# sriramelango/optimized-diffusion-model

Measured on AMD Instinct MI355X. Metric: trajectories/sec (1000-step PC sampler, NCSN++ [1,9,9], bs=128/GPU), higher is better.
Workload: dtype f32; 1 GPU; NCSN++ nf=64 ch_mult=[1,2,2] on [128,1,9,9] per GPU, 1000-step reflected PC sampler (predictor euler_maruyama, corrector none), classifier-free guidance on (2B-sample forwards), fp32; global_batch=128, num_scales=1000, score_evals_per_traj=999, parallelism=single GPU

## Files before the change

### optimized-diffusion-model_amd/csrc/misc_kernels.h

```cpp
#pragma once
#include "common.h"

struct PackJob {
    const float* src;
    float* dst;
    int Cin, Cout;
    int Kpad;
    int Npad;
    int n_off;
    int ntap;
    long s_co, s_ci, s_t;
    int kind;
    const float* src2;
    int col_il;
};

__global__ __launch_bounds__(RDMI_THREADS) void pack_kernel(const PackJob* __restrict__ jobs) {
    const PackJob j = jobs[blockIdx.y];
    const int stride = gridDim.x * RDMI_THREADS;
    if (j.kind == 1) {
        for (int i = blockIdx.x * RDMI_THREADS + threadIdx.x; i < j.Cout; i += stride) j.dst[j.n_off + i] = j.src[i];
        return;
    }
    if (j.kind == 4) {
// ... 201 lines not shown
};

__global__ __launch_bounds__(RDMI_THREADS) void em_update_kernel(
    const float* __restrict__ x, const float* __restrict__ score, const float* __restrict__ zbase,
    const float* __restrict__ t_vec, const float* __restrict__ ts, const StepState* __restrict__ st,
    float* __restrict__ x_out, float* __restrict__ x_mean_out, float* __restrict__ trace,
    int B, int E, int N, float smin, float ratio, float gconst, int z_by_draw) {
    const long i = (long)blockIdx.x * RDMI_THREADS + threadIdx.x;
    if (i >= (long)B * E) return;
    const float t = t_vec ? t_vec[i / E] : ts[st->step];
    const float sigma = smin * powf(ratio, t);
    const float g = sigma * gconst;
    const float dt = -1.0f / (float)N;
    const float* z = z_by_draw ? zbase + (long)st->draw * B * E : zbase;
    const float drift = 0.0f - (g * g) * score[i];
    const float xm = x[i] + drift * dt;
    const float xn = xm + (g * sqrtf(-dt)) * z[i];
    const float xr = reflect_f(xn);
    x_out[i] = xr;
    if (x_mean_out) x_mean_out[i] = reflect_f(xm);
    if (trace) trace[(long)st->step * B * E + i] = xr;
}

__global__ __launch_bounds__(RDMI_THREADS) void em_fused_kernel(
    const float* __restrict__ x, const float* __restrict__ s, const float* __restrict__ w, const float* __restrict__ z,
    float* __restrict__ x_out, float* __restrict__ trace, const float* __restrict__ teacher,
    int B, int E, int N, float t, float smin, float ratio, float gconst, int use_cfg, uint64_t seed, uint64_t elem_offset, uint32_t draw) {
    const long i = (long)blockIdx.x * RDMI_THREADS + threadIdx.x;
    if (i >= (long)B * E) return;
    float score = s[i];
    if (use_cfg) { const float wt = w ? w[i / E] : 0.f; score = (1.0f + wt) * score - wt * s[(long)B * E + i]; }
    float zz;
    if (z) zz = z[i];
    else { const uint64_t g = elem_offset + (uint64_t)i; zz = philox_normal4(seed, g >> 2, draw)[(int)(g & 3)]; }
    const float sigma = smin * powf(ratio, t);
    const float g_ = sigma * gconst;
    const float dt = -1.0f / (float)N;
    const float drift = 0.0f - (g_ * g_) * score;
    const float xm = x[i] + drift * dt;
    const float xr = reflect_f(xm + (g_ * sqrtf(-dt)) * zz);
    if (trace) trace[i] = xr;
    x_out[i] = teacher ? teacher[i] : xr;
}

__global__ __launch_bounds__(64) void langevin_prep_kernel(
    const float* __restrict__ s, const float* __restrict__ w, const float* __restrict__ z_in, float* __restrict__ score_out,
    float* __restrict__ z_out, float* __restrict__ norms, int B, int E, int use_cfg, uint64_t seed, uint64_t elem_offset, uint32_t draw) {
    const int b = blockIdx.x, lane = threadIdx.x;
    const float wt = (use_cfg && w) ? w[b] : 0.f;
    float s2 = 0.f, z2 = 0.f;
    for (int e = lane; e < E; e += 64) {
        const long i = (long)b * E + e;
        float sc = s[i];
        if (use_cfg) sc = (1.0f + wt) * sc - wt * s[(long)B * E + i];
        float zz;
        if (z_in) zz = z_in[i];
        else { const uint64_t g = elem_offset + (uint64_t)i; zz = philox_normal4(seed, g >> 2, draw)[(int)(g & 3)]; }
        score_out[i] = sc; z_out[i] = zz;
        s2 += sc * sc; z2 += zz * zz;
    }
    for (int m = 32; m >= 1; m >>= 1) { s2 += __shfl_xor(s2, m); z2 += __shfl_xor(z2, m); }
    if (lane == 0) { norms[b] = sqrtf(s2); norms[B + b] = sqrtf(z2); }
}
// ... 211 lines not shown
```

### optimized-diffusion-model_amd/csrc/rdmi.hip

```cpp
#include <hip/hip_runtime.h>

#include <algorithm>
#include <cmath>
#include <cstdarg>
#include <cstdio>
#include <cstdlib>
#include <cstring>
#include <climits>
#include <map>
#include <memory>
#include <stdexcept>
#include <string>
#include <vector>

#include "../../include/rdmi.h"
#include "attn_kernel.h"
#include "conv_kernel.h"
#include "misc_kernels.h"
#include "unet_kernel.h"
#include "bwd_kernels.h"
#include "opt_kernels.h"
#include "ode_kernels.h"
#include "tiled_kernels.h"

// ... 119 lines not shown
    dev_ptr<float> d_w;
    size_t w_floats = 0;
    dev_ptr<int> d_int;
    dev_ptr<float> ws;
    size_t ws_per_sample = 0;
    size_t w_t0 = 0, w_t2 = 0, w_dense = 0, b_dense = 0;
    dev_ptr<float> d_h1, d_temb, d_dense;
    dev_ptr<float> d_s2, d_score, d_z, d_norms, d_ts, d_tvec;
    dev_ptr<float> d_tt, d_th1; int tt_cap = 0;
    dev_ptr<float> d_dense_all; size_t dense_all_cap = 0;
    dev_ptr<StepState> d_state;
    bool use_fused = true;
    dev_ptr<long long> d_stamps;
    struct FPatch { int op; int field; std::string param; size_t arena_off; };
    struct FusedProg {
        int S = 1; bool ok = false; std::string why;
        std::vector<FOp> fprog;
        std::vector<FPatch> fpatch; std::vector<short> ftabs;
        std::vector<std::string> fdesc;
        dev_ptr<FOp> d_fprog; dev_ptr<short> d_ftabs; dev_ptr<float> d_spill; size_t spill_per_sample = 0;
        UnetArgs fargs{}; size_t fused_lds = 0;
        bool coop = false; int n_xchg = 0; dev_ptr<unsigned long long> d_xbuf; dev_ptr<int> d_coop_err; int max_nb = 0;
        bool train = false;
    };
    std::unique_ptr<TiledPlan> tiled;
    bool in_train_forward = false;
    dev_ptr<bf16_t> d_w16;
    std::vector<FusedProg> progs;
    int s_min_wg = 256;
    bool use_coop = true;
    int coop_stride = 1;
    unsigned coop_epoch = 0;
    int last_prog = 0;
    const FusedProg* pick(int NB) const {
        if (use_coop) for (auto& q : progs) if (q.ok && q.coop && !q.train && NB <= q.max_nb) return &q;
        const FusedProg* best = nullptr;
        for (auto& q : progs) if (q.ok && !q.coop && !q.train && (q.S == 1 || NB >= s_min_wg * q.S) && (!best || q.S > best->S)) best = &q;
        return best;
    }
    bool fused_ready() const { return !progs.empty() && progs[0].ok; }
    float train_drop_p = 0.f; const unsigned long long* train_seed_dev = nullptr;
    int train_prog = -1;
    std::map<std::string, size_t> wmap;
    bool packed_valid = false;
    bool debug_taps = false;
    bool profiling = false;
    std::vector<ProfEntry> prof;
    std::vector<std::pair<hipEvent_t, hipEvent_t>> ev_pool;
    std::vector<int> ev_entry;
    size_t ev_used = 0;
    std::unique_ptr<TrainPlan> train;
    ~rdmi_ctx();
};

namespace {
// ... 978 lines not shown

int resident_workgroups() {
#ifdef RDMI_EMU
    return 256;
#else
    int dev = 0, cus = 0;
    if (hipGetDevice(&dev) != hipSuccess || hipDeviceGetAttribute(&cus, hipDeviceAttributeMultiprocessorCount, dev) != hipSuccess) return 0;
    return cus;
#endif
}

int build_fused_program(rdmi_ctx* c) {
    if (int e = build_one_program(c, 1)) return e;
    const char* only = std::getenv("RDMI_S");
    if (const char* e = std::getenv("RDMI_S_MIN_WG")) c->s_min_wg = std::max(1, atoi(e));
    for (int S : {2, 4})
        if (c->progs[0].ok && c->arch.n_levels >= 2 && c->max_batch >= c->s_min_wg * S && (!only || atoi(only) >= S))
            if (int e = build_one_program(c, S)) return e;
    if (const char* e = std::getenv("RDMI_COOP")) c->use_coop = atoi(e) != 0;
#ifdef RDMI_EMU
    c->coop_stride = 1;
#endif
    if (const char* e = std::getenv("RDMI_COOP_STRIDE")) c->coop_stride = std::max(1, atoi(e));
    if (c->progs[0].ok && c->use_coop && c->arch.n_levels >= 2 && !only)
        if (int e = build_one_program(c, 4, true)) return e;
    return 0;
}

int build_fused_program_pass(rdmi_ctx* c, rdmi_ctx::FusedProg& q, int S, int TAB_RESERVE, int TAB1_RESERVE, int* tab_used, int* tab1_used, bool coop, bool train) {
    using LT = FusedBuilder::LT;
    const rdmi_arch& a = c->arch;
    q.S = S; q.train = train;
    FusedBuilder b{c, q};
    b.S = S; b.coop = coop; b.train = train;
    if (train) {
        for (size_t i = 0; i < c->tensors.size(); ++i) b.lp_tensor[c->tensors[i].name] = (int)i;
        for (size_t i = 0; i < c->ops.size(); ++i) b.lp_op[c->ops[i].name] = (int)i;
    }
    const int nslot0 = coop ? 1 : S;
    Layout L = build_layout(c);
    std::map<std::string, int> dense_off;
    {
        int dt = 0;
        for (auto& d : L.down) { dense_off[d.name] = dt; dt += d.cout; }
        dense_off["mid_block1"] = dt; dt += L.mid_ch;
        dense_off["mid_block2"] = dt; dt += L.mid_ch;
// ... 213 lines not shown
        FOp& o = q.fprog[(size_t)f.op];
        float* p = q.d_spill.get() + f.off * (size_t)spill_n;
        if (f.which == 1) o.b_g = p; else if (f.which == 2) o.a_g = p; else o.g_out = p;
    }
    UnetArgs& fa = q.fargs;
    fa = UnetArgs{};
    fa.prog = q.d_fprog.get(); fa.nops = (int)q.fprog.size();
    fa.tabs = q.d_ftabs.get(); fa.tab_bytes = (int)(tab0_shorts * sizeof(short)); fa.tab_base = 0;
    if (loadtab_idx >= 0) q.fprog[(size_t)loadtab_idx].a_g = reinterpret_cast<const float*>(q.d_ftabs.get() + tab0_shorts);
    fa.zero_off = TAB_RESERVE; fa.zero_bytes = zero_bytes;
    fa.dense = c->d_dense.get(); fa.dense_stride = c->dense_total; fa.S = S;
    fa.out_elems = c->H * c->W * a.channels;
    if (coop) {
        const int groups_max = ceil_div(coop_max_nb, 4);
        const size_t xb = (size_t)groups_max * 2 * 4 * (size_t)b.xslot_granules * sizeof(unsigned long long);
        HIP_OK(hip_alloc(q.d_xbuf, std::max<size_t>(xb, 16) / sizeof(unsigned long long)));
        HIP_OK(hipMemset(q.d_xbuf.get(), 0, std::max<size_t>(xb, 16)));
        HIP_OK(hip_alloc(q.d_coop_err, 4));
        HIP_OK(hipMemset(q.d_coop_err.get(), 0, 16));
        fa.coop = 1; fa.coop_stride = c->coop_stride; fa.xbuf = q.d_xbuf.get(); fa.xslot = b.xslot_granules;
        fa.coop_err = q.d_coop_err.get();
        if (const char* e = std::getenv("RDMI_COOP_TEST_BREAK")) fa.coop_break = atoi(e);
        q.coop = true; q.n_xchg = b.n_xchg; q.max_nb = coop_max_nb;
    }
    q.fused_lds = (size_t)b.high_water;
    if (const char* e = std::getenv("RDMI_UDBG")) fa.dbg = atoi(e);
    if (std::getenv("RDMI_STAMPS") && (S == 1 || coop)) {
        if (!c->d_stamps) HIP_OK(hip_alloc(c->d_stamps, 1024 + 200 * 8 + 8));
        if (q.fprog.size() > 200) return fail("RDMI_STAMPS: program of %zu ops", q.fprog.size());
        fa.stamps = c->d_stamps.get();
    }
    q.fdesc.clear();
    for (auto& o : q.fprog) {
        char buf[160];
        const char* kn[] = {"GATHER", "STORE", "GN", "CONV", "ATTN", "LOADTAB", "XCHG"};
        if (o.kind == FOP_CONV) snprintf(buf, sizeof buf, "CONV rows=%d mtiles=%d K=%dx%d(+%d) Cout=%d dst=%d%s", o.rows, o.mtiles, o.ntap, o.main_ph.nch * 16, o.nsc ? o.sc[0].nch * 16 : 0, o.Cout, o.dst_kind, o.gn_off >= 0 ? (o.gn_raw ? (o.coop ? " +GN(copy) coop" : " +GN(copy)") : (o.coop ? " +GN coop" : " +GN")) : (o.coop ? " coop" : ""));
        else snprintf(buf, sizeof buf, "%s rows=%d C=%d", kn[o.kind], o.rows, o.C);
        q.fdesc.push_back(buf);
    }
    q.ok = true;
    return 0;
}

struct ProfScope {
    rdmi_ctx* c; hipStream_t s; int entry = -1; size_t slot = 0;
    ProfScope(rdmi_ctx* c_, hipStream_t s_, const std::string& name, double flops) : c(c_), s(s_) {
// ... 116 lines not shown
                case FusedBuilder::F_BIAS2: o.bias2 = p; break;
                case FusedBuilder::F_W: o.main_ph.w = p; break;
                case FusedBuilder::F_SC0W: o.sc[0].w = p; break;
                case FusedBuilder::F_SC1W: o.sc[1].w = p; break;
            }
        }
        HIP_OK(hipMemcpyAsync(q.d_fprog.get(), q.fprog.data(), q.fprog.size() * sizeof(FOp), hipMemcpyHostToDevice, s));
    }
    if (c->fused_ready()) HIP_OK(hipStreamSynchronize(s));
    c->packed_valid = true;
    return 0;
}

struct FwdIn {
    const float* x; int x_mod;
    const float* sig; int sig_mod;
    float t_scalar;
    int t_is_time; float smin, ratio;
    const float* labels; int label_rows;
    float* out; int NB;
    const float* tt_row = nullptr;
    const float* dense_rows = nullptr;
    float drop_p = 0.f; const unsigned long long* seed_dev = nullptr;
};

}
#include "tiled_plan.h"
namespace {

int run_forward(rdmi_ctx* c, const FwdIn& f, hipStream_t s) {
    const rdmi_arch& a = c->arch;
    if (f.NB < 1 || f.NB > c->max_batch) return fail("batch %d outside [1, %d] (rdmi_create max_batch)", f.NB, c->max_batch);
    if (a.scale_by_sigma && !c->tiled) return fail("scale_by_sigma=True is only built for the tiled plan (the shipped GTO-Halo config sets it False, RD/configs/model/ncsnpp.yaml)");
    if (a.conditional && !f.labels) return fail("class_labels is required: the model is conditional (label_emb) -- reference raises here too (RD/models/ncsnpp.py:262)");
    const int T = c->temb, Np_t = (T + 63) & ~63, Np_d = (c->dense_total + 63) & ~63;
    if (!f.tt_row && !f.dense_rows) {
    LinArgs l{};
    l.M = f.NB; l.fourW = P(c, "time_embed.W"); l.nfour = a.nf;
    l.X = f.sig; l.x_mod = f.sig_mod > 0 ? f.sig_mod : f.NB; l.t_is_time = f.t_is_time; l.smin = f.smin; l.ratio = f.ratio;
    l.use_scalar = f.sig ? 0 : 1; l.t_scalar = f.t_scalar;
    l.pre = 2; l.K = pad16(2 * a.nf); l.W = c->d_w.get() + c->w_t0; l.Npad = Np_t; l.N = T; l.bias = P(c, "time_mlp.0.bias");
    l.Y = c->d_h1.get(); l.ldy = T;
    {
        ProfScope ps(c, s, "linear_mfma(time_mlp.0)", 2.0 * f.NB * T * 2 * a.nf);
        hipLaunchKernelGGL(linear_mfma_kernel<1>, dim3((unsigned)ceil_div(f.NB, 16), (unsigned)(Np_t / 64)), dim3(RDMI_THREADS), 0, s, l);
    }
// ... 18 lines not shown
        ProfScope ps(c, s, "linear_mfma(Dense_0 x all)", 2.0 * f.NB * T * c->dense_total);
        hipLaunchKernelGGL((linear_mfma_kernel<1, 16>), dim3((unsigned)ceil_div(f.NB, 16), (unsigned)(Np_d / 64)), dim3(RDMI_THREADS), 0, s, l3);
    }
    }
    HIP_OK(hipGetLastError());
    if (a.compute_dtype == 1 && !c->tiled && !c->in_train_forward)
        return fail("compute_dtype=bf16 on this shape is built for the TRAINING step only (model.train_dtype = 'bf16'); sampling and evaluation of the "
                    "GTO-Halo model run the exact-fp32 plans");
    if (c->tiled) return run_tiled(c, f, s);
    const rdmi_ctx::FusedProg* fq = (c->use_fused && !c->debug_taps) ? c->pick(f.NB) : nullptr;
    if (c->in_train_forward) {
        static const int fused_upto = [] { const char* e = std::getenv("RDMI_TRAIN_FUSED_UPTO"); return e ? atoi(e) : 2 * std::max(resident_workgroups(), 1); }();
        fq = (c->train_prog >= 0 && c->progs[(size_t)c->train_prog].ok && f.NB <= fused_upto) ? &c->progs[(size_t)c->train_prog] : nullptr;
    }
    if (fq) {
        static bool attr_set = false;
        if (!attr_set) {
            HIP_OK(hipFuncSetAttribute(reinterpret_cast<const void*>(unet_wg_kernel<false>), hipFuncAttributeMaxDynamicSharedMemorySize, 160 * 1024));
            HIP_OK(hipFuncSetAttribute(reinterpret_cast<const void*>(unet_wg_kernel<true>), hipFuncAttributeMaxDynamicSharedMemorySize, 160 * 1024));
            HIP_OK(hipFuncSetAttribute(reinterpret_cast<const void*>((unet_wg_kernel<false, true>)), hipFuncAttributeMaxDynamicSharedMemorySize, 160 * 1024));
            HIP_OK(hipFuncSetAttribute(reinterpret_cast<const void*>((unet_wg_kernel<false, true, true>)), hipFuncAttributeMaxDynamicSharedMemorySize, 160 * 1024));
            HIP_OK(hipFuncSetAttribute(reinterpret_cast<const void*>((unet_wg_kernel<true, true, true>)), hipFuncAttributeMaxDynamicSharedMemorySize, 160 * 1024));
            HIP_OK(hipFuncSetAttribute(reinterpret_cast<const void*>((unet_wg_kernel<false, false, false, true>)), hipFuncAttributeMaxDynamicSharedMemorySize, 160 * 1024));
            attr_set = true;
        }
        UnetArgs ua = fq->fargs;
        ua.x_in = f.x; ua.x_mod = f.x_mod; ua.out = f.out; ua.NB = f.NB;
        unsigned nwg = (unsigned)ceil_div(f.NB, fq->S);
        if (fq->coop) {
            nwg = (unsigned)(ceil_div(ceil_div(f.NB, 4), ua.coop_stride) * 4 * ua.coop_stride);
            ua.epoch_base = c->coop_epoch;
            c->coop_epoch += (unsigned)fq->n_xchg;
            if (c->coop_epoch > 0xfff00000u) c->coop_epoch = 0;
        }
        if (f.dense_rows) ua.dense = f.dense_rows;
        double fl = 0;
        for (auto& op : c->ops) fl += op.flops_per_sample;
        ProfScope ps(c, s, "unet_wg_kernel", fl * f.NB);
        c->last_prog = (int)(fq - c->progs.data());
        if (fq->train) {
            ua.drop_p = c->train_drop_p; ua.seed_dev = c->train_seed_dev;
            hipLaunchKernelGGL((unet_wg_kernel<false, false, false, true>), dim3(nwg), dim3(UW_THREADS), fq->fused_lds, s, ua);
            HIP_OK(hipGetLastError());
            return 0;
        }
        if ((ua.stamps || ua.dbg) && fq->S == 1) hipLaunchKernelGGL(unet_wg_kernel<true>, dim3(nwg), dim3(UW_THREADS), fq->fused_lds, s, ua);
        else if ((ua.stamps || ua.dbg) && fq->coop) hipLaunchKernelGGL((unet_wg_kernel<true, true, true>), dim3(nwg), dim3(UW_THREADS), fq->fused_lds, s, ua);
        else if (fq->coop) hipLaunchKernelGGL((unet_wg_kernel<false, true, true>), dim3(nwg), dim3(UW_THREADS), fq->fused_lds, s, ua);
        else if (fq->S > 1) hipLaunchKernelGGL((unet_wg_kernel<false, true>), dim3(nwg), dim3(UW_THREADS), fq->fused_lds, s, ua);
        else hipLaunchKernelGGL(unet_wg_kernel<false>, dim3(nwg), dim3(UW_THREADS), fq->fused_lds, s, ua);
        HIP_OK(hipGetLastError());
        return 0;
    }
    for (auto& op : c->ops) {
        if (op.kind == OP_CONV) {
            ConvArgs ca = op.conv;
            ca.NB = f.NB;
            if (op.a_is_input) { ca.srcA = f.x; ca.srcA_mod = f.x_mod; }
            if (op.out_is_output) ca.out = f.out;
            if (op.use_dense && f.dense_rows) ca.dense = f.dense_rows;
            ProfScope ps(c, s, cfg_name(op.cfg), op.flops_per_sample * f.NB);
            if (int e = launch_conv(op.cfg, ca, s)) return e;
        } else {
            AttnArgs aa = op.attn;
            aa.NB = f.NB;
            ProfScope ps(c, s, "attn_mfma<64>", op.flops_per_sample * f.NB);
            if (int e = launch_attn(aa, s)) return e;
        }
    }
// ... 60 lines not shown
    if (it == c->wmap.end()) return fail("no packed tensor '%s'", key);
    if (it->second + numel > c->w_floats) return fail("packed tensor '%s': %zu floats exceed the arena", key, numel);
    HIP_OK(hipMemcpyAsync(dst, c->d_w.get() + it->second, numel * sizeof(float), hipMemcpyDeviceToDevice, (hipStream_t)stream));
    return 0;
}

const char* rdmi_path_info(rdmi_ctx* c) {
    static thread_local std::string s;
    if (!c) return "";
    if (c->tiled) {
        s = std::string("tiled (") + (c->arch.compute_dtype == 1 ? "bf16 MFMA operands, fp32 accumulate" : "fp32") + "): " + std::to_string(c->tiled->launches.size()) + " launches over HBM-resident NHWC tensors (" + std::to_string(c->tiled->ws_per_sample * 4 / 1024) + " KiB of activations per sample)";
        long n_resize = 0;
        for (auto& l : c->tiled->launches) n_resize += std::holds_alternative<TResizeL>(l.op);
        s += "; resize launches (h onto an odd skip grid): " + std::to_string(n_resize);
    } else if (c->fused_ready() && c->use_fused && !c->debug_taps) {
        s = "fused: workgroup-resident U-Net, " + std::to_string(c->progs[0].fprog.size()) + " ops, " + std::to_string(c->progs[0].fused_lds) + " B LDS";
        for (size_t i = 1; i < c->progs.size(); ++i)
            if (c->progs[i].coop)
                s += c->progs[i].ok ? "; co-operative groups of 4 workgroups up to batch " + std::to_string(c->progs[i].max_nb) + " (" + std::to_string(c->progs[i].fprog.size()) + " ops, " + std::to_string(c->progs[i].n_xchg) + " exchanges, id stride " + std::to_string(c->coop_stride) + (c->use_coop ? ")" : ", disabled)")
                                    : "; co-operative program unavailable (" + c->progs[i].why + ")";
            else
            s += c->progs[i].ok ? "; S=" + std::to_string(c->progs[i].S) + " samples/workgroup from batch " + std::to_string(c->s_min_wg * c->progs[i].S) + " (" + std::to_string(c->progs[i].fprog.size()) + " ops)"
                                : "; S=" + std::to_string(c->progs[i].S) + " unavailable (" + c->progs[i].why + ")";
    } else {
        s = "layers: " + std::to_string(c->ops.size()) + " launches" + (c->fused_ready() ? "" : " (fused unavailable: " + (c->progs.empty() ? std::string("not built") : c->progs[0].why) + ")");
    }
    for (auto& q : c->progs) if (q.train && !q.ok) s += "; fused training forward unavailable (" + q.why + ")";
    if (c->train_prog >= 0 && c->progs[(size_t)c->train_prog].ok)
        s += "; training forward: fused program (" + std::to_string(c->progs[(size_t)c->train_prog].fprog.size()) + " ops, layer outputs stashed for the backward)";
    if (c->train) s += "; input-gradient backward calls: " + std::to_string(c->train->input_dgrad_calls);
    return s.c_str();
}

int rdmi_philox_normal(float* z, size_t n, unsigned long long seed, unsigned long long elem_offset, unsigned draw, void* stream) {
    if (n == 0) return 0;
    if (!z) return fail("null argument");
    hipLaunchKernelGGL(philox_normal_kernel, dim3((unsigned)((n + 4 * RDMI_THREADS - 1) / (4 * RDMI_THREADS))), dim3(RDMI_THREADS), 0, (hipStream_t)stream, z, (long)n,
                       (uint64_t)seed, (uint64_t)elem_offset, (const int*)nullptr, (int)draw);
    HIP_OK(hipGetLastError());
    return 0;
}

int rdmi_coop_status(rdmi_ctx* c, int* gave_up) {
    if (!c || !gave_up) return fail("null argument");
    *gave_up = 0;
    for (auto& q : c->progs)
// ... 256 lines not shown
    if (c->dense_all_cap < (size_t)U * dense_row_floats) {
        c->dense_all_cap = 0;
        HIP_OK(hip_alloc(c->d_dense_all, (size_t)U * dense_row_floats));
        c->dense_all_cap = (size_t)U * dense_row_floats;
    }
    auto dense_chunk = [&](int i0) -> int {
        const int u = std::min(U, nupd - i0);
        LinArgs l3{};
        l3.M = u * NBm; l3.X = c->d_tt.get() + (size_t)i0 * T; l3.ldx = T; l3.pre = 3; l3.K = T; l3.row_div = NBm;
        if (a.conditional && labels) { l3.labels = labels; l3.Wl = P(c, "label_emb.weight"); l3.ncls = a.num_classes; l3.label_rows = B; }
        l3.W = c->d_w.get() + c->w_dense; l3.Npad = Np_d; l3.N = c->dense_total;
        l3.bias = c->d_w.get() + c->b_dense; l3.Y = c->d_dense_all.get(); l3.ldy = c->dense_total;
        ProfScope ps(c, s, "linear_mfma(Dense_0 x all, chunk of updates)", 2.0 * l3.M * T * c->dense_total);
        hipLaunchKernelGGL((linear_mfma_kernel<1, 16>), dim3((unsigned)ceil_div(l3.M, 16), (unsigned)(Np_d / 64)), dim3(RDMI_THREADS), 0, s, l3);
        HIP_OK(hipGetLastError());
        return 0;
    };
    auto net_eval = [&](int i, float t) -> int {
        FwdIn f{x, o->use_cfg ? B : 0, nullptr, 0, t, 1, smin, ratio, labels, B, c->d_s2.get(), NBm};
        f.tt_row = c->d_tt.get() + (size_t)i * T;
        f.dense_rows = c->d_dense_all.get() + (size_t)(i % U) * dense_row_floats;
        return run_forward(c, f, s);
    };
    uint32_t draw = 0;
    for (int i = 0; i < o->N - 1; ++i) {
        const float t = ts[(size_t)i];
        if (i % U == 0) { if (int e = dense_chunk(i)) return e; }
        if (o->corrector == 1) {
            for (int k = 0; k < o->n_steps_each; ++k, ++draw) {
                if (int e = net_eval(i, t)) return e;
                ProfScope ps(c, s, "langevin_update", 0);
                hipLaunchKernelGGL(langevin_prep_kernel, dim3((unsigned)B), dim3(64), 0, s, (const float*)c->d_s2.get(), weight,
                                   noise ? noise + (size_t)draw * BE : (const float*)nullptr, c->d_score.get(), c->d_z.get(), c->d_norms.get(), B, E,
                                   o->use_cfg, (uint64_t)o->seed, eoff, draw);
                hipLaunchKernelGGL(langevin_update_kernel, dim3(gBE), dim3(RDMI_THREADS), 64, s, (const float*)x,
                                   (const float*)c->d_score.get(), (const float*)c->d_z.get(), (const float*)c->d_norms.get(), (const StepState*)nullptr, x,
                                   (float*)nullptr, B, E, o->snr, 0);
            }
        }
        if (int e = net_eval(i, t)) return e;
        {
            ProfScope ps(c, s, "em_fused", 0);
            hipLaunchKernelGGL(em_fused_kernel, dim3(gBE), dim3(RDMI_THREADS), 0, s, (const float*)x, (const float*)c->d_s2.get(), weight,
                               noise ? noise + (size_t)draw * BE : (const float*)nullptr, x, trace ? trace + (size_t)i * BE : (float*)nullptr,
                               teacher ? teacher + (size_t)i * BE : (const float*)nullptr, B, E, o->N, t, smin, ratio, gc, o->use_cfg,
                               (uint64_t)o->seed, eoff, draw);
            ++draw;
        }
        HIP_OK(hipGetLastError());
        if (c->profiling && (i % 16 == 15)) prof_collect(c);
// ... 253 lines not shown
```

### optimized-diffusion-model_amd/csrc/unet_kernel.h

```cpp
#pragma once
#include <cstddef>

#include "common.h"

#define UW_THREADS 512
#define UW_WAVES 8
#ifndef UW_PF_M4
#define UW_PF_M4 4
#endif
#ifndef UW_PF_N1
#define UW_PF_N1 4
#endif
#ifndef UW_PF_KS1
#define UW_PF_KS1 4
#endif
#ifndef UW_PRIO
#define UW_PRIO 0
#endif
#ifndef UW_LIGHT_BARRIER
#define UW_LIGHT_BARRIER 0
#endif

__device__ __forceinline__ void lds_barrier() {
#if defined(__HIP_DEVICE_COMPILE__) && UW_LIGHT_BARRIER
// ... 54 lines not shown
struct UnetArgs {
    const FOp* prog; int nops;
    const short* tabs; int tab_bytes;
    int tab_base;
    int zero_off;
    int zero_bytes;
    const float* dense; int dense_stride;
    const float* x_in; int x_mod;
    float* out;
    int NB;
    int S;
    int dbg;
    long long* stamps;
    int coop, coop_stride;
    unsigned long long* xbuf;
    int xslot;
    unsigned epoch_base;
    int out_elems;
    float drop_p; const unsigned long long* seed_dev;
    int* coop_err;
    int coop_break;
};

struct OpW { int w0, w1; };
static_assert(sizeof(FOp) <= 512, "FOp must fit two VGPRs per wave");
__device__ __forceinline__ int opw_at(const OpW& r, int word) {
    return word < 64 ? __builtin_amdgcn_readlane(r.w0, word) : __builtin_amdgcn_readlane(r.w1, word - 64);
}
#define OPI(r, field) opw_at(r, (int)(offsetof(FOp, field) / 4))
#define OPF(r, field) __builtin_bit_cast(float, OPI(r, field))
#define OPP(r, T, field) \
    reinterpret_cast<T*>((unsigned long long)(unsigned)opw_at(r, (int)(offsetof(FOp, field) / 4)) | ((unsigned long long)(unsigned)opw_at(r, (int)(offsetof(FOp, field) / 4) + 1) << 32))
__device__ __forceinline__ OpW opw_load(const FOp* op, int lane) {
    OpW r;
    constexpr int NW = (int)(sizeof(FOp) / 4);
    const int* g = reinterpret_cast<const int*>(op);
    r.w0 = lane < NW ? __builtin_bit_cast(int, ldg1(reinterpret_cast<const float*>(g + lane))) : 0;
    r.w1 = lane + 64 < NW ? __builtin_bit_cast(int, ldg1(reinterpret_cast<const float*>(g + lane + 64))) : 0;
    return r;
}

__device__ __forceinline__ float* lds_f(int off) { return reinterpret_cast<float*>(rdmi_lds + off); }

__device__ __forceinline__ int samp_of(int samp, int hw_shift, int row) { return samp >= 0 ? samp : (row >> hw_shift); }

template <bool MS>
// ... 877 lines not shown
#pragma unroll
            for (int r = 0; r < 4; ++r) v[r] = (v[r] + add_all + rv[r]) * o_scale;
        } else {
#pragma unroll
            for (int r = 0; r < 4; ++r) v[r] = (v[r] + add_all + 0.f) * o_scale;
        }
        if (!fused_gn || OPI(w, gn_raw) != 0) {
            float* p = dstp + (size_t)row0 * drs + col;
#pragma unroll
            for (int r = 0; r < 4; ++r) p[r * drs] = v[r];
        }
        if (fused_gn) {
            const float s1 = quad_sum((v[0] + v[1]) + (v[2] + v[3])), s2 = quad_sum((v[0] * v[0] + v[1] * v[1]) + (v[2] * v[2] + v[3] * v[3]));
            const float mean = s1 * OPF(w, inv_cnt);
            const float rstd = (1.0f / sqrtf(fmaxf(s2 * OPF(w, inv_cnt) - mean * mean, 0.f) + OPF(w, eps))) * gmul;
            const int act = OPI(w, gn_act), grs = OPI(w, gn_rs);
            float* p = lds_f(OPI(w, gn_off)) + (size_t)row0 * grs + col;
#pragma unroll
            for (int r = 0; r < 4; ++r) { const float y = (v[r] - mean) * rstd + gadd; p[r * grs] = act ? silu_f(y) : y; }
        }
    }
}

__device__ __forceinline__ void fop_xchg(const OpW& w, const UnetArgs& u, int g, int m, int tid, int* failw) {
    const int mode = OPI(w, a_hw), rows = OPI(w, rows), Cs = OPI(w, C), xi = OPI(w, xidx);
    const int d_off = OPI(w, dst_off), d_rs = OPI(w, dst_rs), s_off = OPI(w, src_off), s_rs = OPI(w, src_rs);
    const int a_off = OPI(w, a_off), a_rs = OPI(w, a_rs);
    const unsigned epoch = u.epoch_base + (unsigned)xi + 1u;
    const int csh = 31 - __builtin_clz((unsigned)Cs);
    const int half = (rows << csh) >> 1;
    const int np = s_off >= 0 ? 2 * half : half;
    const unsigned slotb = (unsigned)u.xslot * 8u;
    const unsigned gbase = (unsigned)((g * 2 + (xi & 1)) * 4) * slotb;
    const XBuf xb = xbuf_make(u.xbuf, 0x7fffffffu);
    auto at = [&](int p, int j) -> int {
        const int sel = p >= half ? 1 : 0, i = (p - sel * half) << 1, row = i >> csh, c = i & (Cs - 1);
        if (mode == 0) return ((sel ? s_off : d_off) >> 2) + row * (sel ? s_rs : d_rs) + j * Cs + c;
        return (d_off >> 2) + (j * rows + row) * d_rs + c;
    };
    typedef float f32x2 __attribute__((vector_size(8)));
    constexpr int KMAX = 1;
    const bool withhold = u.coop_break != 0 && g == 0 && m == 3 && xi == 0;
#pragma unroll
    for (int k = 0; k < KMAX; ++k) {
        const int p = tid + k * UW_THREADS;
        if (p < np && !withhold) {
            f32x2 v;
            if (mode == 0) v = *reinterpret_cast<const f32x2*>(lds_f(0) + at(p, m));
            else {
                const int i = p << 1, row = i >> csh, c = i & (Cs - 1);
                v = *reinterpret_cast<const f32x2*>(lds_f(a_off) + row * a_rs + c);
                *reinterpret_cast<f32x2*>(lds_f(0) + at(p, m)) = v;
            }
            const float v0 = v[0], v1 = v[1];
            xbuf_store16(xb, gbase + (unsigned)m * slotb + (unsigned)p * 16u, __builtin_bit_cast(unsigned, v0), __builtin_bit_cast(unsigned, v1), epoch);
        }
// ... 13 lines not shown
            }
        bool ok = true;
#pragma unroll
        for (int k = 0; k < KMAX; ++k)
            if (k < nk) {
#pragma unroll
                for (int jj = 0; jj < 3; ++jj) { const unsigned t1 = y[k * 3 + jj][1], t3 = y[k * 3 + jj][3]; ok &= t1 == epoch && t3 == epoch; }
            }
        if (ok) break;
        if (++spins > RDMI_SPIN_LIMIT) { *failw = 1; __hip_atomic_store(u.coop_err, 1, __ATOMIC_RELAXED, __HIP_MEMORY_SCOPE_AGENT); break; }
        spin_relax();
    }
#pragma unroll
    for (int k = 0; k < KMAX; ++k) {
        const int p = tid + k * UW_THREADS;
        if (!broken && k < nk && p < np) {
#pragma unroll
            for (int jj = 0; jj < 3; ++jj) {
                const unsigned a = y[k * 3 + jj][0], b = y[k * 3 + jj][2];
                *reinterpret_cast<f32x2*>(lds_f(0) + at(p, (m + 1 + jj) & 3)) = f32x2{__builtin_bit_cast(float, a), __builtin_bit_cast(float, b)};
            }
        }
    }
}

__device__ __forceinline__ void fop_attn(const OpW& w, int wave, int lane) {
    struct { int L, Lpad, q_off, k_off, vt_off, p_off, qk_rs, k_rs, ps, C, dst_off, dst_rs; float att_scale; } o;
    o.L = OPI(w, L); o.Lpad = OPI(w, Lpad); o.q_off = OPI(w, q_off); o.k_off = OPI(w, k_off); o.vt_off = OPI(w, vt_off); o.p_off = OPI(w, p_off);
    o.qk_rs = OPI(w, qk_rs); o.k_rs = OPI(w, k_rs); o.ps = OPI(w, ps); o.C = OPI(w, C); o.dst_off = OPI(w, dst_off); o.dst_rs = OPI(w, dst_rs); o.att_scale = OPF(w, att_scale);
    const int lrow = lane & 15, kq = lane >> 4;
    const int L = o.L, mtiles = o.Lpad >> 4;
    const float* Q = lds_f(o.q_off);
    const float* K = lds_f(o.k_off);
    const float* Vt = lds_f(o.vt_off);
    float* P = lds_f(o.p_off);
    const int rs = o.qk_rs, krs = o.k_rs, ps = o.ps;
    const int nchq = o.C >> 4;
    for (int mt = wave; mt < mtiles; mt += UW_WAVES) {
        f32x4 s[6];
#pragma unroll
        for (int t = 0; t < 6; ++t) s[t] = f32x4{0.f, 0.f, 0.f, 0.f};
        const int qrow = min(mt * 16 + lrow, L - 1);
        for (int ch = 0; ch < nchq; ++ch) {
            const f32x4 af = *reinterpret_cast<const f32x4*>(Q + (size_t)qrow * rs + ch * 16 + kq * 4);
#pragma unroll
            for (int t = 0; t < 6; ++t) {
// ... 48 lines not shown
#pragma unroll
                    for (int j = 0; j < 4; ++j) acc[i] = mfma16(af[j], bf[j], acc[i]);
                }
            }
        }
        float* O = lds_f(o.dst_off);
        const float* b3 = OPP(w, const float, bias);
        const int o_resid = OPI(w, resid_off), o_resid_rs = OPI(w, resid_rs);
        const float o_scale = OPF(w, scale), badd = b3 ? ldg1(b3 + col) : 0.f;
#pragma unroll
        for (int i = 0; i < 3; ++i) {
            const int mt = wm + 2 * i;
            if (mt < mtiles)
                for (int r = 0; r < 4; ++r) {
                    const int row = mt * 16 + kq * 4 + r;
                    if (row < L) {
                        float v = acc[i][r];
                        if (b3) v = (v + badd + lds_f(o_resid)[(size_t)row * o_resid_rs + col]) * o_scale;
                        O[(size_t)row * o.dst_rs + col] = v;
                    }
                }
        }
    }
}

template <bool DIAG, bool MS = false, bool COOP = false, bool TRAIN = false>
__global__ __launch_bounds__(UW_THREADS) void unet_wg_kernel(UnetArgs u) {
    const int tid = threadIdx.x, lane = tid & 63;
    const int wave = __builtin_amdgcn_readfirstlane(tid >> 6);
    int n = MS ? blockIdx.x * u.S : blockIdx.x, n_multi = n, n_spill = n, spill_cap = u.NB;
    int cg = 0, cm = 0;
    if (COOP) {
        const int st = u.coop_stride, bid = blockIdx.x, blk = bid / (4 * st), r = bid - blk * 4 * st;
        cm = r / st; cg = blk * st + (r - cm * st);
        if (cg * 4 >= u.NB) return;
        n = min(cg * 4 + cm, u.NB - 1);
        n_multi = cg * 4;
        n_spill = bid * 4; spill_cap = 0x7fffffff;
    }
    {
        const int nw = u.tab_bytes >> 2;
        const int* src = reinterpret_cast<const int*>(u.tabs);
        int* dst = reinterpret_cast<int*>(rdmi_lds + u.tab_base);
        for (int i = tid; i < nw; i += UW_THREADS) dst[i] = src[i];
        float* z = lds_f(u.zero_off);
        for (int i = tid; i < (u.zero_bytes >> 2); i += UW_THREADS) z[i] = 0.f;
// ... 30 lines not shown
                else fop_conv<DIAG, MS && !COOP, TRAIN>(cur, u, multi ? n_multi : n, wave, lane, fine);
                break;
            case FOP_ATTN: fop_attn(cur, wave, lane); break;
            case FOP_LOADTAB: {
                const int* src = OPP(cur, const int, a_g);
                int* dst = reinterpret_cast<int*>(rdmi_lds + OPI(cur, dst_off));
                const int nw = OPI(cur, rows) >> 2;
                for (int i = tid; i < nw; i += UW_THREADS) dst[i] = src[i];
                break;
            }
            case FOP_XCHG: if (COOP) fop_xchg(cur, u, cg, cm, tid, failw); break;
            default: break;
        }
        if (kind == FOP_STORE || (kind == FOP_CONV && OPI(cur, dst_kind) == 2)) __syncthreads();
        else lds_barrier();
        if (DIAG && u.stamps && n == 0 && tid == 0) u.stamps[pc + 1] = clock64();
        cur = nxt; nxt = nn; pgm = ngm; pbt = nbt;
    }
    if (COOP && *failw) {
        const int E = (int)u.out_elems;
        for (int i = tid; i < E; i += UW_THREADS) u.out[(size_t)n * E + i] = __builtin_nanf("");
    }
}
```

Before: 184.4 trajectories/s.

## Run multiple sampler steps inside one resident co-operative UNet kernel launch

Adds a persistent loop kernel that runs the fused co-operative UNet forward and the Euler-Maruyama update for many sampler steps inside a single launch. Workgroups exchange cond/uncond scores through a global epoch-tagged pair buffer for classifier-free guidance. The per-step host launches of the forward and update kernels go away, along with the round trip of x through separate kernels. In exchange it adds spin-wait synchronisation between workgroups, extra buffers, and a restriction to predictor-only seeded runs with no trace or teacher.

```diff
diff --git a/optimized-diffusion-model_amd/csrc/misc_kernels.h b/optimized-diffusion-model_amd/csrc/misc_kernels.h
--- a/optimized-diffusion-model_amd/csrc/misc_kernels.h
+++ b/optimized-diffusion-model_amd/csrc/misc_kernels.h
@@ -247,23 +247,31 @@
     if (trace) trace[(long)st->step * B * E + i] = xr;
 }
 
+__device__ __forceinline__ float em_fused_elem(float xv, float s_c, float s_u, float wt, int use_cfg, const float* zp, uint64_t seed, uint64_t g,
+                                               uint32_t draw, int N, float t, float smin, float ratio, float gconst) {
+#pragma clang fp contract(off)
+    float score = s_c;
+    if (use_cfg) score = (1.0f + wt) * score - wt * s_u;
+    float zz;
+    if (zp) zz = *zp;
+    else zz = philox_normal4(seed, g >> 2, draw)[(int)(g & 3)];
+    const float sigma = smin * powf(ratio, t);
+    const float g_ = sigma * gconst;
+    const float dt = -1.0f / (float)N;
+    const float drift = __builtin_fmaf(-(g_ * g_), score, 0.0f);
+    const float xm = __builtin_fmaf(drift, dt, xv);
+    return reflect_f(__builtin_fmaf(g_ * sqrtf(-dt), zz, xm));
+}
+
 __global__ __launch_bounds__(RDMI_THREADS) void em_fused_kernel(
     const float* __restrict__ x, const float* __restrict__ s, const float* __restrict__ w, const float* __restrict__ z,
     float* __restrict__ x_out, float* __restrict__ trace, const float* __restrict__ teacher,
     int B, int E, int N, float t, float smin, float ratio, float gconst, int use_cfg, uint64_t seed, uint64_t elem_offset, uint32_t draw) {
     const long i = (long)blockIdx.x * RDMI_THREADS + threadIdx.x;
     if (i >= (long)B * E) return;
-    float score = s[i];
-    if (use_cfg) { const float wt = w ? w[i / E] : 0.f; score = (1.0f + wt) * score - wt * s[(long)B * E + i]; }
-    float zz;
-    if (z) zz = z[i];
-    else { const uint64_t g = elem_offset + (uint64_t)i; zz = philox_normal4(seed, g >> 2, draw)[(int)(g & 3)]; }
-    const float sigma = smin * powf(ratio, t);
-    const float g_ = sigma * gconst;
-    const float dt = -1.0f / (float)N;
-    const float drift = 0.0f - (g_ * g_) * score;
-    const float xm = x[i] + drift * dt;
-    const float xr = reflect_f(xm + (g_ * sqrtf(-dt)) * zz);
+    const float wt = (use_cfg && w) ? w[i / E] : 0.f;
+    const float su = use_cfg ? s[(long)B * E + i] : 0.f;
+    const float xr = em_fused_elem(x[i], s[i], su, wt, use_cfg, z ? z + i : nullptr, seed, elem_offset + (uint64_t)i, draw, N, t, smin, ratio, gconst);
     if (trace) trace[i] = xr;
     x_out[i] = teacher ? teacher[i] : xr;
 }
diff --git a/optimized-diffusion-model_amd/csrc/rdmi.hip b/optimized-diffusion-model_amd/csrc/rdmi.hip
--- a/optimized-diffusion-model_amd/csrc/rdmi.hip
+++ b/optimized-diffusion-model_amd/csrc/rdmi.hip
@@ -165,6 +165,7 @@
         UnetArgs fargs{}; size_t fused_lds = 0;
         bool coop = false; int n_xchg = 0; dev_ptr<unsigned long long> d_xbuf; dev_ptr<int> d_coop_err; int max_nb = 0;
         bool train = false;
+        dev_ptr<unsigned long long> d_pair; dev_ptr<float> d_xin; int pair_slot = 0;
     };
     std::unique_ptr<TiledPlan> tiled;
     bool in_train_forward = false;
@@ -174,6 +175,9 @@
     bool use_coop = true;
     int coop_stride = 1;
     unsigned coop_epoch = 0;
+    unsigned pair_epoch = 0;
+    int loop_last = 0;
+    int loop_updates = -1;
     int last_prog = 0;
     const FusedProg* pick(int NB) const {
         if (use_coop) for (auto& q : progs) if (q.ok && q.coop && !q.train && NB <= q.max_nb) return &q;
@@ -1198,6 +1202,7 @@
     c->coop_stride = 1;
 #endif
     if (const char* e = std::getenv("RDMI_COOP_STRIDE")) c->coop_stride = std::max(1, atoi(e));
+    if (const char* e = std::getenv("RDMI_LOOP_UPDATES")) c->loop_updates = std::max(0, atoi(e));
     if (c->progs[0].ok && c->use_coop && c->arch.n_levels >= 2 && !only)
         if (int e = build_one_program(c, 4, true)) return e;
     return 0;
@@ -1457,6 +1462,11 @@
         fa.coop_err = q.d_coop_err.get();
         if (const char* e = std::getenv("RDMI_COOP_TEST_BREAK")) fa.coop_break = atoi(e);
         q.coop = true; q.n_xchg = b.n_xchg; q.max_nb = coop_max_nb;
+        q.pair_slot = 2 * ((fa.out_elems + 1) / 2);
+        const size_t pg = (size_t)2 * (size_t)std::max(coop_max_nb, 1) * (size_t)q.pair_slot;
+        HIP_OK(hip_alloc(q.d_pair, pg));
+        HIP_OK(hipMemset(q.d_pair.get(), 0, pg * sizeof(unsigned long long)));
+        HIP_OK(hip_alloc(q.d_xin, (size_t)ceil_div(std::max(coop_max_nb, 1), 4) * 4 * (size_t)fa.out_elems));
     }
     q.fused_lds = (size_t)b.high_water;
     if (const char* e = std::getenv("RDMI_UDBG")) fa.dbg = atoi(e);
@@ -1619,6 +1629,7 @@
     const float* tt_row = nullptr;
     const float* dense_rows = nullptr;
     float drop_p = 0.f; const unsigned long long* seed_dev = nullptr;
+    const UnetLoop* loop = nullptr;
 };
 
 }
@@ -1683,6 +1694,7 @@
             HIP_OK(hipFuncSetAttribute(reinterpret_cast<const void*>((unet_wg_kernel<false, true, true>)), hipFuncAttributeMaxDynamicSharedMemorySize, 160 * 1024));
             HIP_OK(hipFuncSetAttribute(reinterpret_cast<const void*>((unet_wg_kernel<true, true, true>)), hipFuncAttributeMaxDynamicSharedMemorySize, 160 * 1024));
             HIP_OK(hipFuncSetAttribute(reinterpret_cast<const void*>((unet_wg_kernel<false, false, false, true>)), hipFuncAttributeMaxDynamicSharedMemorySize, 160 * 1024));
+            HIP_OK(hipFuncSetAttribute(reinterpret_cast<const void*>(unet_loop_kernel), hipFuncAttributeMaxDynamicSharedMemorySize, 160 * 1024));
             attr_set = true;
         }
         UnetArgs ua = fq->fargs;
@@ -1691,13 +1703,23 @@
         if (fq->coop) {
             nwg = (unsigned)(ceil_div(ceil_div(f.NB, 4), ua.coop_stride) * 4 * ua.coop_stride);
             ua.epoch_base = c->coop_epoch;
-            c->coop_epoch += (unsigned)fq->n_xchg;
+            c->coop_epoch += (unsigned)fq->n_xchg * (unsigned)(f.loop ? f.loop->nupd : 1);
             if (c->coop_epoch > 0xfff00000u) c->coop_epoch = 0;
+        }
+        UnetLoop ul{};
+        if (f.loop) {
+            if (!fq->coop || fq->train || ua.stamps || ua.dbg) return fail("resident sampler loop: not the co-operative production program");
+            ul = *f.loop;
+            ul.nx = fq->n_xchg; ul.xin = fq->d_xin.get(); ul.pair = fq->d_pair.get(); ul.pair_slot = fq->pair_slot;
+            ul.pair_epoch = c->pair_epoch;
+            c->pair_epoch += (unsigned)f.loop->nupd;
+            if (c->pair_epoch > 0xfff00000u) c->pair_epoch = 0;
+            ua.x_in = nullptr; ua.x_mod = 0;
         }
         if (f.dense_rows) ua.dense = f.dense_rows;
         double fl = 0;
         for (auto& op : c->ops) fl += op.flops_per_sample;
-        ProfScope ps(c, s, "unet_wg_kernel", fl * f.NB);
+        ProfScope ps(c, s, "unet_wg_kernel", fl * f.NB * (f.loop ? f.loop->nupd : 1));
         c->last_prog = (int)(fq - c->progs.data());
         if (fq->train) {
             ua.drop_p = c->train_drop_p; ua.seed_dev = c->train_seed_dev;
@@ -1705,7 +1727,8 @@
             HIP_OK(hipGetLastError());
             return 0;
         }
-        if ((ua.stamps || ua.dbg) && fq->S == 1) hipLaunchKernelGGL(unet_wg_kernel<true>, dim3(nwg), dim3(UW_THREADS), fq->fused_lds, s, ua);
+        if (f.loop) hipLaunchKernelGGL(unet_loop_kernel, dim3(nwg), dim3(UW_THREADS), fq->fused_lds, s, ua, ul);
+        else if ((ua.stamps || ua.dbg) && fq->S == 1) hipLaunchKernelGGL(unet_wg_kernel<true>, dim3(nwg), dim3(UW_THREADS), fq->fused_lds, s, ua);
         else if ((ua.stamps || ua.dbg) && fq->coop) hipLaunchKernelGGL((unet_wg_kernel<true, true, true>), dim3(nwg), dim3(UW_THREADS), fq->fused_lds, s, ua);
         else if (fq->coop) hipLaunchKernelGGL((unet_wg_kernel<false, true, true>), dim3(nwg), dim3(UW_THREADS), fq->fused_lds, s, ua);
         else if (fq->S > 1) hipLaunchKernelGGL((unet_wg_kernel<false, true>), dim3(nwg), dim3(UW_THREADS), fq->fused_lds, s, ua);
@@ -1812,6 +1835,13 @@
             else
             s += c->progs[i].ok ? "; S=" + std::to_string(c->progs[i].S) + " samples/workgroup from batch " + std::to_string(c->s_min_wg * c->progs[i].S) + " (" + std::to_string(c->progs[i].fprog.size()) + " ops)"
                                 : "; S=" + std::to_string(c->progs[i].S) + " unavailable (" + c->progs[i].why + ")";
+        for (auto& q : c->progs)
+            if (q.coop && q.ok && c->use_coop) {
+                const std::string cap = c->loop_updates > 0 ? "at most " + std::to_string(c->loop_updates) : std::string("one Dense_0 chunk of");
+                s += c->loop_updates == 0 ? "; resident sampler loop off (RDMI_LOOP_UPDATES=0)"
+                                          : "; resident sampler loop on (seeded predictor-only sampling: " + cap + " updates per co-operative launch" +
+                                                (c->loop_last > 0 ? ", " + std::to_string(c->loop_last) + " in the last call)" : ")");
+            }
     } else {
         s = "layers: " + std::to_string(c->ops.size()) + " launches" + (c->fused_ready() ? "" : " (fused unavailable: " + (c->progs.empty() ? std::string("not built") : c->progs[0].why) + ")");
     }
@@ -2114,10 +2144,30 @@
         f.dense_rows = c->d_dense_all.get() + (size_t)(i % U) * dense_row_floats;
         return run_forward(c, f, s);
     };
+    const rdmi_ctx::FusedProg* lq = nullptr;
+    if (o->corrector == 0 && !noise && !trace && !teacher && c->loop_updates != 0 && !c->tiled && c->use_fused && !c->debug_taps && !c->profiling && E <= 2 * UW_THREADS) {
+        const rdmi_ctx::FusedProg* q = c->pick(NBm);
+        if (q && q->coop && !q->fargs.stamps && !q->fargs.dbg) lq = q;
+    }
     uint32_t draw = 0;
     for (int i = 0; i < o->N - 1; ++i) {
         const float t = ts[(size_t)i];
         if (i % U == 0) { if (int e = dense_chunk(i)) return e; }
+        if (lq) {
+            const int u = std::min(std::min(U - i % U, nupd - i), c->loop_updates > 0 ? c->loop_updates : INT_MAX);
+            UnetLoop lp{};
+            if (i == 0) c->loop_last = u;
+            lp.nupd = u; lp.dense_upd_stride = (long long)dense_row_floats; lp.ts = c->d_ts.get() + i; lp.x = x; lp.weight = weight;
+            lp.B = B; lp.use_cfg = o->use_cfg; lp.N = o->N; lp.smin = smin; lp.ratio = ratio; lp.gconst = gc;
+            lp.seed = (unsigned long long)o->seed; lp.elem_offset = eoff; lp.draw0 = draw;
+            FwdIn f{x, o->use_cfg ? B : 0, nullptr, 0, t, 1, smin, ratio, labels, B, c->d_s2.get(), NBm};
+            f.tt_row = c->d_tt.get() + (size_t)i * T;
+            f.dense_rows = c->d_dense_all.get() + (size_t)(i % U) * dense_row_floats;
+            f.loop = &lp;
+            if (int e = run_forward(c, f, s)) return e;
+            draw += (uint32_t)u; i += u - 1;
+            continue;
+        }
         if (o->corrector == 1) {
             for (int k = 0; k < o->n_steps_each; ++k, ++draw) {
                 if (int e = net_eval(i, t)) return e;
diff --git a/optimized-diffusion-model_amd/csrc/unet_kernel.h b/optimized-diffusion-model_amd/csrc/unet_kernel.h
--- a/optimized-diffusion-model_amd/csrc/unet_kernel.h
+++ b/optimized-diffusion-model_amd/csrc/unet_kernel.h
@@ -100,6 +100,22 @@
     int coop_break;
 };
 
+struct UnetLoop {
+    int nupd;
+    int nx;
+    long long dense_upd_stride;
+    const float* ts;
+    float* x;
+    float* xin;
+    const float* weight;
+    unsigned long long* pair;
+    int pair_slot;
+    unsigned pair_epoch;
+    int B, use_cfg, N;
+    float smin, ratio, gconst;
+    unsigned long long seed, elem_offset; unsigned draw0;
+};
+
 struct OpW { int w0, w1; };
 static_assert(sizeof(FOp) <= 512, "FOp must fit two VGPRs per wave");
 __device__ __forceinline__ int opw_at(const OpW& r, int word) {
@@ -1023,7 +1039,8 @@
     }
 }
 
-__device__ __forceinline__ void fop_xchg(const OpW& w, const UnetArgs& u, int g, int m, int tid, int* failw) {
+template <bool SEQ = false>
+__device__ __forceinline__ void fop_xchg(const OpW& w, const UnetArgs& u, int g, int m, int tid, int* failw, int xseq = 0) {
     const int mode = OPI(w, a_hw), rows = OPI(w, rows), Cs = OPI(w, C), xi = OPI(w, xidx);
     const int d_off = OPI(w, dst_off), d_rs = OPI(w, dst_rs), s_off = OPI(w, src_off), s_rs = OPI(w, src_rs);
     const int a_off = OPI(w, a_off), a_rs = OPI(w, a_rs);
@@ -1032,7 +1049,7 @@
     const int half = (rows << csh) >> 1;
     const int np = s_off >= 0 ? 2 * half : half;
     const unsigned slotb = (unsigned)u.xslot * 8u;
-    const unsigned gbase = (unsigned)((g * 2 + (xi & 1)) * 4) * slotb;
+    const unsigned gbase = (unsigned)((g * 2 + ((SEQ ? xi + xseq : xi) & 1)) * 4) * slotb;
     const XBuf xb = xbuf_make(u.xbuf, 0x7fffffffu);
     auto at = [&](int p, int j) -> int {
         const int sel = p >= half ? 1 : 0, i = (p - sel * half) << 1, row = i >> csh, c = i & (Cs - 1);
@@ -1092,6 +1109,32 @@
             }
         }
     }
+}
+
+template <int KMAX, int NJ, class OffF>
+__device__ __forceinline__ bool xchg_wait(const XBuf& xb, const UnetArgs& u, unsigned epoch, int nk, OffF off, u32x4 (&y)[NJ * KMAX], int* failw) {
+    unsigned long long spins = 0;
+    bool broken = __hip_atomic_load(u.coop_err, __ATOMIC_RELAXED, __HIP_MEMORY_SCOPE_AGENT) != 0;
+    if (broken) *failw = 1;
+    for (; !broken;) {
+#pragma unroll
+        for (int k = 0; k < KMAX; ++k)
+            if (k < nk) {
+#pragma unroll
+                for (int jj = 0; jj < NJ; ++jj) y[k * NJ + jj] = xbuf_load16(xb, off(k, jj));
+            }
+        bool ok = true;
+#pragma unroll
+        for (int k = 0; k < KMAX; ++k)
+            if (k < nk) {
+#pragma unroll
+                for (int jj = 0; jj < NJ; ++jj) { const unsigned t1 = y[k * NJ + jj][1], t3 = y[k * NJ + jj][3]; ok &= t1 == epoch && t3 == epoch; }
+            }
+        if (ok) break;
+        if (++spins > RDMI_SPIN_LIMIT) { *failw = 1; __hip_atomic_store(u.coop_err, 1, __ATOMIC_RELAXED, __HIP_MEMORY_SCOPE_AGENT); break; }
+        spin_relax();
+    }
+    return broken;
 }
 
 __device__ __forceinline__ void fop_attn(const OpW& w, int wave, int lane) {
@@ -1186,6 +1229,51 @@
                 }
         }
     }
+}
+
+__device__ __forceinline__ bool loop_update(const UnetArgs& u, const UnetLoop& q, int k, int n, int wgrow, int tid, int* failw) {
+    const int E = u.out_elems, np = (E + 1) >> 1, B = q.B;
+    const bool cfg = q.use_cfg != 0, uncond = cfg && n >= B, dup = wgrow >= u.NB;
+    const int b = uncond ? n - B : n;
+    const int p = min(tid, np - 1), e0 = 2 * p, e1 = min(2 * p + 1, E - 1);
+    const bool mine = tid < np, two = 2 * p + 1 < E;
+    const float* sp = u.out + (size_t)n * E;
+    const float own0 = ldg1(sp + e0), own1 = ldg1(sp + e1);
+    float oth0 = 0.f, oth1 = 0.f;
+    if (cfg) {
+        const unsigned epoch = q.pair_epoch + (unsigned)k + 1u;
+        const unsigned slotb = (unsigned)q.pair_slot * 8u;
+        const unsigned base = (unsigned)((k & 1) * u.NB) * slotb;
+        const XBuf xb = xbuf_make(q.pair, 0x7fffffffu);
+        if (mine && !dup) xbuf_store16(xb, base + (unsigned)n * slotb + (unsigned)p * 16u, __builtin_bit_cast(unsigned, own0), __builtin_bit_cast(unsigned, own1), epoch);
+        const unsigned from = base + (unsigned)(uncond ? n - B : n + B) * slotb + (unsigned)p * 16u;
+        u32x4 y[1];
+        const bool broken = xchg_wait<1, 1>(xb, u, epoch, 1, [&](int, int) { return from; }, y, failw);
+        if (!broken) {
+            const unsigned a = y[0][0], c = y[0][2];
+            oth0 = __builtin_bit_cast(float, a); oth1 = __builtin_bit_cast(float, c);
+        }
+    }
+    __syncthreads();
+    if (*failw) return true;
+    const float wt = (cfg && q.weight) ? ldg1(q.weight + b) : 0.f;
+    const float t = ldg1(q.ts + k);
+    float* xr = q.xin + (size_t)wgrow * E;
+    const uint64_t g0 = q.elem_offset + (uint64_t)b * (uint64_t)E;
+    const unsigned draw = q.draw0 + (unsigned)k;
+    const float x0 = em_fused_elem(ldg1(xr + e0), uncond ? oth0 : own0, uncond ? own0 : oth0, wt, q.use_cfg, nullptr, q.seed, g0 + (uint64_t)e0, draw, q.N, t, q.smin, q.ratio, q.gconst);
+    const float x1 = em_fused_elem(ldg1(xr + e1), uncond ? oth1 : own1, uncond ? own1 : oth1, wt, q.use_cfg, nullptr, q.seed, g0 + (uint64_t)e1, draw, q.N, t, q.smin, q.ratio, q.gconst);
+    if (mine) {
+        stg1(xr + e0, x0);
+        if (two) stg1(xr + e1, x1);
+        if (!uncond && !dup) {
+            float* xc = q.x + (size_t)b * E;
+            stg1(xc + e0, x0);
+            if (two) stg1(xc + e1, x1);
+        }
+    }
+    __syncthreads();
+    return false;
 }
 
 template <bool DIAG, bool MS = false, bool COOP = false, bool TRAIN = false>
@@ -1262,3 +1350,101 @@
         for (int i = tid; i < E; i += UW_THREADS) u.out[(size_t)n * E + i] = __builtin_nanf("");
     }
 }
+
+template <bool DIAG, bool MS, bool COOP, bool TRAIN, bool LOOP>
+__device__ __forceinline__ void unet_wg_body(UnetArgs& u, const UnetLoop* lp) {
+    const int tid = threadIdx.x, lane = tid & 63;
+    const int wave = __builtin_amdgcn_readfirstlane(tid >> 6);
+    int n = MS ? blockIdx.x * u.S : blockIdx.x, n_multi = n, n_spill = n, spill_cap = u.NB;
+    int cg = 0, cm = 0;
+    int wgrow = 0;
+    if (COOP) {
+        const int st = u.coop_stride, bid = blockIdx.x, blk = bid / (4 * st), r = bid - blk * 4 * st;
+        cm = r / st; cg = blk * st + (r - cm * st);
+        if (cg * 4 >= u.NB) return;
+        n = min(cg * 4 + cm, u.NB - 1);
+        n_multi = cg * 4;
+        n_spill = bid * 4; spill_cap = 0x7fffffff;
+        wgrow = cg * 4 + cm;
+    }
+    {
+        const int nw = u.tab_bytes >> 2;
+        const int* src = reinterpret_cast<const int*>(u.tabs);
+        int* dst = reinterpret_cast<int*>(rdmi_lds + u.tab_base);
+        for (int i = tid; i < nw; i += UW_THREADS) dst[i] = src[i];
+        float* z = lds_f(u.zero_off);
+        for (int i = tid; i < (u.zero_bytes >> 2); i += UW_THREADS) z[i] = 0.f;
+    }
+#if defined(__HIP_DEVICE_COMPILE__) && UW_PRIO == 1
+    if (wave >= 4) __builtin_amdgcn_s_setprio(1);
+#elif defined(__HIP_DEVICE_COMPILE__) && UW_PRIO == 2
+    if (wave < 4) __builtin_amdgcn_s_setprio(1);
+#endif
+    float* stat = lds_f(u.zero_off + u.zero_bytes);
+    int* const failw = reinterpret_cast<int*>(stat) + 270;
+    if (COOP && tid == 0) *failw = 0;
+    if (LOOP) {
+        const int E = u.out_elems;
+        const float* xs = lp->x + (size_t)((lp->use_cfg && n >= lp->B) ? n - lp->B : n) * E;
+        float* xr = lp->xin + (size_t)wgrow * E;
+        for (int i = tid; i < E; i += UW_THREADS) stg1(xr + i, ldg1(xs + i));
+        u.x_in = lp->xin + ((ptrdiff_t)wgrow - n) * E;
+        __syncthreads();
+    }
+    if (DIAG && u.stamps && n == 0 && tid == 0) u.stamps[0] = clock64();
+    OpW cur = opw_load(u.prog, lane);
+    OpW nxt = opw_load(u.prog + (u.nops > 1 ? 1 : 0), lane);
+    f32x4 pgm = {1.f, 1.f, 1.f, 1.f}, pbt = {0.f, 0.f, 0.f, 0.f};
+    gn_prefetch(cur, tid, pgm, pbt);
+    int upd = 0;
+    do {
+    for (int pc = 0; pc < u.nops; ++pc) {
+        const OpW nn = opw_load(u.prog + (pc + 2 < u.nops ? pc + 2 : LOOP ? pc + 2 - u.nops : u.nops - 1), lane);
+        long long* fine = (DIAG && u.stamps && n == 0 && tid == ((u.dbg >> 16) & 7) * 64) ? u.stamps + 1024 + pc * 8 : nullptr;
+        const int kind = OPI(cur, kind);
+        if (DIAG && fine) fine[2] = clock64();
+        f32x4 ngm = pgm, nbt = pbt;
+        if (LOOP || pc + 1 < u.nops) gn_prefetch(nxt, tid, ngm, nbt);
+        if (DIAG && fine) fine[3] = clock64();
+        const int skip = (DIAG && u.dbg) ? ((kind == FOP_GN ? 4 : kind == FOP_CONV ? 8 : kind == FOP_ATTN ? 16 : 32) & u.dbg) : 0;
+        const bool multi = MS && OPI(cur, samp) < 0;
+        switch (skip ? -1 : kind) {
+            case FOP_GATHER: fop_gather<MS>(cur, u, multi ? n_spill : n, multi ? spill_cap : u.NB, COOP ? cm : 0, tid); break;
+            case FOP_STORE: fop_store<MS>(cur, u, multi ? n_spill : n, multi ? spill_cap : u.NB, tid); break;
+            case FOP_GN: fop_gn<MS>(cur, stat, tid, pgm, pbt, DIAG ? u.dbg : 0); break;
+            case FOP_CONV:
+                if (COOP && OPI(cur, coop)) fop_conv_coop<DIAG>(cur, u, n_multi, cm, wave, lane, fine);
+                else fop_conv<DIAG, MS && !COOP, TRAIN>(cur, u, multi ? n_multi : n, wave, lane, fine);
+                break;
+            case FOP_ATTN: fop_attn(cur, wave, lane); break;
+            case FOP_LOADTAB: {
+                const int* src = OPP(cur, const int, a_g);
+                int* dst = reinterpret_cast<int*>(rdmi_lds + OPI(cur, dst_off));
+                const int nw = OPI(cur, rows) >> 2;
+                for (int i = tid; i < nw; i += UW_THREADS) dst[i] = src[i];
+                break;
+            }
+            case FOP_XCHG: if (COOP) fop_xchg<true>(cur, u, cg, cm, tid, failw, upd * lp->nx); break;
+            default: break;
+        }
+        if (kind == FOP_STORE || (kind == FOP_CONV && OPI(cur, dst_kind) == 2)) __syncthreads();
+        else lds_barrier();
+        if (DIAG && u.stamps && n == 0 && tid == 0) u.stamps[pc + 1] = clock64();
+        cur = nxt; nxt = nn; pgm = ngm; pbt = nbt;
+    }
+    if (LOOP) {
+        if (loop_update(u, *lp, upd, n, wgrow, tid, failw)) break;
+        u.dense += lp->dense_upd_stride; u.epoch_base += (unsigned)lp->nx;
+    }
+    } while (LOOP && ++upd < lp->nupd);
+    if (COOP && *failw) {
+        const int E = (int)u.out_elems;
+        for (int i = tid; i < E; i += UW_THREADS) u.out[(size_t)n * E + i] = __builtin_nanf("");
+        if (LOOP) {
+            const int b = (lp->use_cfg && n >= lp->B) ? n - lp->B : n;
+            for (int i = tid; i < E; i += UW_THREADS) { lp->xin[(size_t)wgrow * E + i] = __builtin_nanf(""); lp->x[(size_t)b * E + i] = __builtin_nanf(""); }
+        }
+    }
+}
+
+__global__ __launch_bounds__(UW_THREADS) void unet_loop_kernel(UnetArgs u, UnetLoop lp) { unet_wg_body<false, true, true, false, true>(u, &lp); }
```

Result: no change. 185.1 trajectories/s, median of 6 (+0.4%).
